# HuiGuanLab/Lite-MKD

Hardware: AMD Instinct MI355X
Metric: episodes/sec (5-way 5-shot, 8x224^2 frames) (higher is better)
Workload: dtype f32

## Files before the change

include/lmkd.h:

```cpp
#ifndef LMKD_H
#define LMKD_H
#ifdef __cplusplus
extern "C" {
#endif

int lmkd_abi_version(void);
const char* lmkd_last_error(void);
int lmkd_device_check(int device);
int lmkd_set_activation_dtype(int mode);
int lmkd_get_activation_dtype(void);

int lmkd_gemm_f32(char layA, char layB, int M, int N, int K, float alpha, const float* A, long lda, long sA,
                  const float* B, long ldb, long sB, float beta, float* C, long ldc, long sC, const float* bias,
                  int relu, int batch, void* stream);
int lmkd_gemm_set_mode(int mode);
int lmkd_gemm_set_tile(int t);
long lmkd_gemm_ticket_words(void);
int lmkd_gemm_f32_splitk(char layA, char layB, int M, int N, int K, float alpha, const float* A, long lda, long sA,
                         const float* B, long ldb, long sB, float beta, float* C, long ldc, long sC, const float* bias,
                         int relu, int batch, void* workspace, long ws_bytes, unsigned* tickets, void* stream);

long lmkd_conv2d_packed_weight_elems(int Cout, int Cin, int Cs, int KH, int KW, int mode);
int lmkd_conv2d_pack_weights(const float* w_oihw, float* wp, int Cout, int Cin, int Cs, int KH, int KW, int mode ,
                             void* stream);
int lmkd_conv2d_fwd_row_tiles(int N, int H, int W, int Cout, int KH, int KW, int stride, int pad);
int lmkd_conv2d_fwd_row_tiles_cs(int N, int H, int W, int Cs, int Cout, int KH, int KW, int stride, int pad);
int lmkd_set_elementwise_wg_per_cu(int n);
int lmkd_conv_set_compute_dtype(int mode);
typedef struct lmkd_amax_desc {
  const void* x_words;
  const void* dy_words;
  void* out_words;
  const void* ref_words;
  int flags;
} lmkd_amax_desc;
#define LMKD_AMAX_FENCED 1
int lmkd_h2_fence_eval(const void* const* words, void* const* refs, int n, int* flags, void* stream);
long lmkd_conv_h2_fallbacks(void);
int lmkd_amax(const float* x, long n, void* word, void* stream);
long lmkd_amax_words(void);
long lmkd_conv2d_plane_elems(int ncols, int Kp);
long lmkd_conv_h2_launches(void);
int lmkd_conv2d_repack_multi(const float* const* ws, void* const* wfs, const int* dims, int n, void* stream);
int lmkd_conv2d_split_weights(const float* wp, void* wf, int ncols, int Kp, void* stream);
int lmkd_conv_get_compute_dtype(void);
int lmkd_conv_set_wgrad_planes(int on);
int lmkd_conv_set_patch(int on);
int lmkd_conv_set_stem_patch(int on);
int lmkd_conv_set_s2_patch(int on);
int lmkd_conv_set_wgrad_win16(int on);
int lmkd_conv_set_wgrad_stem(int on);
int lmkd_conv_set_wgrad_window(int on);
int lmkd_conv_set_patch16(int on);
int lmkd_conv_set_persistent(int on);
int lmkd_conv_set_xcd_mode(int mode);
int lmkd_conv_set_tile(int id);
int lmkd_conv2d_fwd(const float* x, const float* wp_fwd, float* y, float* stat_partial, int N, int H, int W, int Cs, int Cout,
                    int KH, int KW, int stride, int pad, void* stream);
int lmkd_conv2d_fwd_pre(const float* x_raw, const float* pre_stats, const float* wp_fwd, float* y, float* stat_partial, int N, int H,
                        int W, int Cs, int Cout, int KH, int KW, int stride, int pad, void* stream);
int lmkd_conv2d_fwd_bn(const float* x, const float* wp_fwd, float* y, const float* bn_stats, const float* res , int relu,
                       int N, int H, int W, int Cs, int Cout, int KH, int KW, int stride, int pad, void* stream,
                       const lmkd_amax_desc* amax );
int lmkd_conv2d_bwd_data(const float* dy, const float* wp_dgrad, float* dx, int N, int H, int W, int Cin, int Cout, int KH, int KW,
                         int stride, int pad, int accumulate, void* stream);
int lmkd_conv2d_bwd_data_bn_tiles(int N, int H, int W, int Cin, int Cout, int KH, int KW, int stride, int pad);
int lmkd_conv2d_bwd_data_bn(const float* dy, const float* wp_dgrad, float* dx, const float* bn_x, const float* bn_stats, float* part,
                            int N, int H, int W, int Cin, int Cout, int KH, int KW, int stride, int pad, void* stream);
long lmkd_conv2d_bwd_weight_workspace(int N, int H, int W, int Cs, int Cout, int KH, int KW, int stride, int pad);
int lmkd_conv2d_bwd_weight(const float* x, const float* dy, float* dw_oihw, float* workspace, long ws_bytes, int N, int H, int W,
                           int Cs, int Cin, int Cout, int KH, int KW, int stride, int pad, void* stream);
int lmkd_conv2d_bwd_weight_pre(const float* x_raw, const float* pre_stats, const float* dy, float* dw_oihw, float* workspace,
                               long ws_bytes, int N, int H, int W, int Cs, int Cin, int Cout, int KH, int KW, int stride, int pad,
                               void* stream);

int lmkd_conv2d_plan(int kind, int N, int H, int W, int Cs, int Cin, int Cout, int KH, int KW, int stride, int pad, int* info_host);

int lmkd_conv2d_bwd_weight_acc(const float* x, const float* pre_stats, const float* dy, float* dw_oihw, float* workspace, long ws_bytes,
                               int N, int H, int W, int Cs, int Cin, int Cout, int KH, int KW, int stride, int pad, void* stream);

int lmkd_frames_u8_to_nhwc4(const unsigned char* src, float* dst, const int* crop_y, const int* crop_x, const int* flip, int F, int Hs,
                            int Ws, int H, int W, int frames_per_video, void* stream);
int lmkd_resize_plan(int in_size, int out_size, int* bounds_host, int* coeffs_host);
int lmkd_resize_pass_u8(const unsigned char* src, unsigned char* dst, const int* bounds_dev, const int* coeffs_dev, int ksize, long outer,
                        int n_in, int n_out, long inner, void* stream);
int lmkd_frames_resize_crop_nhwc4(const unsigned char* src, float* dst, const int* bounds_h, const int* coeffs_h, int ksize_h,
                                  const int* bounds_v, const int* coeffs_v, int ksize_v, const int* crop_y, const int* crop_x,
                                  const int* flip, int F, int Hs, int Ws, int Hr, int Wr, int H, int W, int frames_per_video, void* stream);
long lmkd_jpeg_desc_bytes(void);
long lmkd_jpeg_pool_bytes(int n);
const char* lmkd_jpeg_reason(int reason);
int lmkd_jpeg_plan(const unsigned char* data, const long long* offsets, int n, void* descs, void* pool, long pool_cap, long long* info,
                   long long* totals);
int lmkd_jpeg_decode(const unsigned char* data, const void* descs, const void* pool, int n, short* coef, unsigned char* planes,
                     unsigned char* out, int* status, long long max_blocks, long long max_pixels, void* stream);
int lmkd_jpeg_decode_host(const unsigned char* data, const void* descs, const void* pool, int n, short* coef, unsigned char* planes,
                          unsigned char* out, int* status);
int lmkd_nchw3_to_nhwc4(const float* x_nchw, float* y_nhwc4, int N, int H, int W, void* stream, void* amax_words);
long lmkd_ticket_words(void);
int lmkd_bn_finalize(const float* partial, int T, int C, long count, const float* gamma, const float* beta, float* running_mean,
                     float* running_var, float momentum, float eps, float* stats, double* scratch, unsigned* tickets, void* stream,
                     const lmkd_amax_desc* amax );
int lmkd_bn_running_update(float* running_mean, float* running_var, const float* stats, int C, float momentum, void* stream);
int lmkd_bn_running_update_multi(float* const* running_mean, float* const* running_var, const float* const* stats_first,
                                 const float* const* stats_second, const int* C, int n, float momentum, void* stream);
int lmkd_bn_running_update_multi_nbt(float* const* running_mean, float* const* running_var, const float* const* stats_first,
                                     const float* const* stats_second, long long* const* num_batches_tracked, const int* C, int n,
                                     float momentum, void* stream);
int lmkd_bn_eval_stats(int C, const float* gamma, const float* beta, const float* running_mean, const float* running_var, float eps,
                       float* stats, void* stream);
int lmkd_bn_apply(const float* x, const float* stats, const float* res, const float* rstats, float* y, long rows, int C, int relu,
                  int res_mode, unsigned* mask_bits, void* stream);
long lmkd_bn_bwd_workspace(int C);
int lmkd_bn_backward(const float* dy, const float* x, const float* yact, const float* stats, const float* gamma, float* dx,
                     float* g_out, float* dgamma, float* dbeta, float* coef, void* workspace, unsigned* tickets, long rows, int C,
                     int mask_mode, int accumulate_param_grads, void* stream);
int lmkd_bn_backward_part(const float* part, int T, const float* dy, const float* x, const float* stats, const float* gamma, float* dx,
                          float* dgamma, float* dbeta, float* coef, void* workspace, unsigned* tickets, long rows, int C,
                          int accumulate_param_grads, void* stream);
int lmkd_relu_backward(const float* dy, const float* y, float* g, long n, void* stream);
int lmkd_bn_relu_maxpool_fwd(const float* x, const float* stats, float* y, unsigned char* idx, float* cmax, int N, int H, int W, int C,
                             void* stream);
int lmkd_maxpool_bwd(const float* dy, const unsigned char* idx, float* g, int N, int H, int W, int C, void* stream);
int lmkd_bn_backward_stats(const float* dy, const float* cmax, const float* stats, const float* gamma, float* dgamma, float* dbeta,
                           float* coef, void* workspace, unsigned* tickets, long pooled_rows, long count, int C, int accumulate_param_grads,
                           void* stream);
int lmkd_stem_unpool_bn_bwd(const float* dy, const unsigned char* idx, const float* c, const float* stats, const float* coef, float* dc,
                            int N, int H, int W, int C, void* stream, const lmkd_amax_desc* amax );
int lmkd_adaptive_maxpool_mean_fwd(const float* x, float* y, int F, int H, int W, int C, void* stream);
int lmkd_adaptive_maxpool_mean_bwd(const float* x, const float* dy, float* dx, int F, int H, int W, int C, void* stream);
long lmkd_colsum_workspace(int C);
// ... 151 lines not shown
```

lite-mkd_amd/csrc/conv.hip:

```cpp
#include "gemm_core.h"
#include <atomic>
#include <mutex>

struct ConvGemmArgs {
  const float* src;
  const float* wpk;
  float* out;
  float* stat_partial;
  int N, Hs, Ws, Cs;
  int Hr, Wr, rows_per_class, tiles_per_class;
  int sh;
  int Ho, Wo, Co, omul;
  int Kp, cps, nclass;
  int n_rt, n_ct, xcd_mode;
  int taps_pm1;
  int grid_step;
  int grid_total;
  int same;
  int halo;
  int accum;
  const float* ep_stats;
  const float* ep_res;
  int ep_relu;
  const float* pre_stats;
// ... 701 lines not shown
  return pr.multiProcessorCount;
}
static int g_conv_persist = 1;
extern "C" int lmkd_conv_set_persistent(int on) { g_conv_persist = on ? 1 : 0; return LMKD_OK; }
template <auto K>
static int persistent_grid(int threads, size_t lds, int total) {
  if (!g_conv_persist) return total;
  static PersistOcc c;
  int occ = 0;
  {
    std::lock_guard<std::mutex> lk(c.mu);
    const int n = c.n.load();
    for (int i = 0; i < n; ++i) if (c.lds[i] == (int)lds) occ = c.occ[i];
    if (!occ) {
      if (hipOccupancyMaxActiveBlocksPerMultiprocessor(&occ, K, threads, lds) != hipSuccess || occ < 1) occ = 1;
      if (n < 8) { c.lds[n] = (int)lds; c.occ[n] = occ; c.n.store(n + 1); }
    }
  }
  const int slots = occ * lmkd_cu_count();
  if (total <= slots) return total;
  const int rounds = cdiv(total, slots);
  const int g = (cdiv(total, rounds) + 7) & ~7;
  return g < total ? g : total;
}

static int g_conv_patch = 1;
extern "C" int lmkd_conv_set_patch(int on) { g_conv_patch = on ? 1 : 0; return LMKD_OK; }
static int patch_halo(const ConvGemmArgs& a) {
  if (!g_conv_patch || !conv_planes() || a.Cs % 32 != 0 || a.sh != 1) return -1;
  const bool plain = a.nclass == 1 && a.Hs == a.Ho && a.Ws == a.Wo;
  const bool classes = a.nclass == 4 && a.Hr == a.Hs && a.Wr == a.Ws;
  if (!plain && !classes) return -1;
  int halo = 0;
  for (int c = 0; c < a.nclass; ++c)
    for (int t = 0; t < a.ntap[c]; ++t) {
      const int sft = a.taps[c][t].dh * a.Ws + a.taps[c][t].dw;
      halo = std::max(halo, sft < 0 ? -sft : sft);
    }
  return halo <= PATCH_HALO_MAX ? halo : -1;
}
static inline bool conv_same_size(int H, int W, int KH, int KW, int stride, int pad) {
  return g_conv_patch && stride == 1 && conv_out(H, KH, stride, pad) == H && conv_out(W, KW, stride, pad) == W && (KH / 2) * W + KW / 2 <= PATCH_HALO_MAX;
}

static int g_conv_s2_patch = 1;
extern "C" int lmkd_conv_set_s2_patch(int on) { g_conv_s2_patch = on ? 1 : 0; return LMKD_OK; }
static int g_patch16 = 1;
extern "C" int lmkd_conv_set_patch16(int on) { g_patch16 = on < 0 ? 0 : (on > 2 ? 2 : on); return LMKD_OK; }

#ifdef LMKD_STAMPS
extern "C" int lmkd_debug_stamps(unsigned long long* host, int zero) {
  if (zero) {
    void* p = nullptr;
    if (hipGetSymbolAddress(&p, HIP_SYMBOL(g_lmkd_stamps)) != hipSuccess) return LMKD_EHIP;
    return hipMemset(p, 0, sizeof(g_lmkd_stamps)) == hipSuccess ? LMKD_OK : LMKD_EHIP;
  }
  return hipMemcpyFromSymbol(host, HIP_SYMBOL(g_lmkd_stamps), sizeof(g_lmkd_stamps)) == hipSuccess ? LMKD_OK : LMKD_EHIP;
}
#endif
static inline int taps_within_one(const ConvGemmArgs& a) {
  for (int c = 0; c < a.nclass; ++c)
    for (int t = 0; t < a.ntap[c]; ++t)
      if (a.taps[c][t].dh < -1 || a.taps[c][t].dh > 1 || a.taps[c][t].dw < -1 || a.taps[c][t].dw > 1) return 0;
  return 1;
}

static bool fwd_s2_patch_ok(int N, int H, int W, int Cs, int Cout, int KH, int KW, int stride, int pad) {
  if (!(g_conv_s2_patch && g_patch16 && g_conv_patch && conv_nprod(g_lmkd_act_bf16) >= 6) || Cs % 32 != 0 || stride != 2 || KH != 3 ||
      KW != 3 || pad != 1 || H % 2 != 0 || W % 2 != 0 || W / 2 + 1 > PATCH_HALO_MAX)
    return false;
  const int id = pick_conv_cfg((long)N * (H / 2) * (W / 2), 1, Cout, true);
  return id == 11 || id == 12;
}

static int g_conv_stem_patch = 1;
extern "C" int lmkd_conv_set_stem_patch(int on) { g_conv_stem_patch = on ? 1 : 0; return LMKD_OK; }
static int stem_patch_pitch(int W, int Cs, int Cout, int KH, int KW, int stride, int pad) {
  if (!g_conv_stem_patch || !conv_planes() || Cs != 4 || KH != 7 || KW != 7 || stride != 2 || pad != 3 || Cout > 64) return 0;
  const int Wo = conv_out(W, KW, stride, pad);
  int wp = std::max(2 * Wo + 6, W + 3);
  wp += wp & 1;
  return (2 * Wo <= 256 && wp <= STEM_MAX_WP) ? wp : 0;
}

enum class ConvFam : unsigned char {
  Tile,
  Gather,
  Patch,
  Patch16,
  Patch1p,
  Stem,
};
enum ConvIO : unsigned char { IO_PLAIN, IO_PRE, IO_EP, IO_ACT16, IO_BNB };
struct ConvPlan {
  ConvFam fam;
  unsigned char io;
  bool src2;
  bool smallc;
  bool bnb_form;
  bool amax_pass;
  int stats;
  int tile;
  int nprod;
  int nclass, xcd;
  int halo;
  int seg_m0, seg_t0, tiles_per_class, n_rt, n_ct;
  int grid;
  int lds;
};

static void fwd_geometry(ConvGemmArgs& a, int N, int H, int W, int Cs, int Cout, int KH, int KW, int stride, int pad, int seg_n0) {
  memset(&a, 0, sizeof(a));
  const int KWp = kw_padded(Cs, KW);
  a.N = N; a.Hs = H; a.Ws = W; a.Cs = Cs;
  a.Ho = conv_out(H, KH, stride, pad); a.Wo = conv_out(W, KW, stride, pad); a.Co = Cout;
  a.Hr = a.Ho; a.Wr = a.Wo; a.rows_per_class = N * a.Ho * a.Wo; a.tiles_per_class = cdiv(a.rows_per_class, 128);
  a.seg_m0 = seg_n0 * a.Ho * a.Wo;
  a.sh = stride; a.omul = 1; a.nclass = 1;
  a.Kp = KH * KWp * Cs;
  a.div_hw = make_fastdiv(a.Hr * a.Wr); a.div_w = make_fastdiv(a.Wr);
  if (Cs == 4) {
    a.cps = 1;
    if (KH > LMKD_MAX_TAPS) return;
    a.ntap[0] = KH;
    for (int kh = 0; kh < KH; ++kh) a.taps[0][kh] = Tap{kh - pad, -pad, kh * KWp * Cs};
  } else {
    a.cps = Cs / 32;
    if (KH * KW > LMKD_MAX_TAPS) return;
    a.ntap[0] = KH * KW;
    for (int kh = 0; kh < KH; ++kh)
      for (int kw = 0; kw < KW; ++kw) a.taps[0][kh * KW + kw] = Tap{kh - pad, kw - pad, (kh * KWp + kw) * Cs};
  }
}

static void dgrad_geometry(ConvGemmArgs& a, int N, int H, int W, int Cin, int Cout, int KH, int KW, int stride, int pad, int seg_n0) {
  memset(&a, 0, sizeof(a));
  const int Ho = conv_out(H, KH, stride, pad), Wo = conv_out(W, KW, stride, pad);
  a.N = N; a.Hs = Ho; a.Ws = Wo; a.Cs = Cout;
  a.Ho = H; a.Wo = W; a.Co = Cin;
  a.Kp = KH * KW * Cout; a.cps = Cout / 32;
  a.sh = 1;
  const bool fits = KH * KW <= LMKD_MAX_TAPS;
  if (stride == 1) {
    a.nclass = 1; a.omul = 1; a.Hr = H; a.Wr = W;
    int nt = 0;
    for (int kh = 0; kh < KH && fits; ++kh)
      for (int kw = 0; kw < KW; ++kw) a.taps[0][nt++] = Tap{pad - kh, pad - kw, (kh * KW + kw) * Cout};
    a.ntap[0] = nt;
  } else {
    a.nclass = 4; a.omul = 2; a.Hr = (H + 1) / 2; a.Wr = (W + 1) / 2;
    for (int c = 0; c < 4 && fits; ++c) {
      const int ph = c >> 1, pw = c & 1;
      int nt = 0;
      for (int kh = 0; kh < KH; ++kh) {
        if (((ph + pad - kh) & 1) != 0) continue;
        for (int kw = 0; kw < KW; ++kw) {
          if (((pw + pad - kw) & 1) != 0) continue;
          const int nh = ph + pad - kh, nw = pw + pad - kw;
          a.taps[c][nt++] = Tap{nh >= 0 ? nh / 2 : -((-nh) / 2), nw >= 0 ? nw / 2 : -((-nw) / 2), (kh * KW + kw) * Cout};
        }
      }
      a.ntap[c] = nt;
    }
  }
  a.rows_per_class = N * a.Hr * a.Wr;
  a.seg_m0 = seg_n0 * a.Hr * a.Wr;
  a.tiles_per_class = cdiv(a.rows_per_class, 128);
  a.div_hw = make_fastdiv(a.Hr * a.Wr); a.div_w = make_fastdiv(a.Wr);
}

static ConvPlan plan_conv(const ConvGemmArgs& a, int halo, bool same, bool smallc, int stats, bool src2) {
  ConvPlan p;
  memset(&p, 0, sizeof(p));
  const bool act16 = g_lmkd_act_bf16;
  const int ncols = a.Co;
  p.io = a.ep_stats ? IO_EP : act16 ? IO_ACT16 : a.pre_stats ? IO_PRE : a.bnb_x ? IO_BNB : IO_PLAIN;
  p.src2 = src2; p.smallc = smallc; p.stats = stats; p.nclass = a.nclass; p.halo = halo;
  int id = pick_conv_cfg(a.rows_per_class, a.nclass, ncols, same);
  if (conv_planes() && !(stats == 2 && smallc)) {
    if (halo < 0) {
      id = id == 10 || id == 13 || id == 14 ? 7 : (id == 11 ? 9 : (id == 12 ? 8 : id));
      p.fam = ConvFam::Gather;
      p.nprod = conv_nprod(act16);
    } else if (id == 13 || id == 14) {
      p.fam = ConvFam::Patch1p;
      p.nprod = 1;
    } else {
      const bool h2 = conv_nprod(act16, a.h2_xw && !a.ep_stats) == 3;
      const bool h2_on_32 = g_patch16 == 1 && id == 11 && ncols <= 64 && h2 && !src2;
      const bool p16 = (id == 11 || id == 12) && g_patch16 && conv_nprod(act16) >= 6;
      p.bnb_form = p16 && a.nclass == 1 && ncols % 4 == 0;
      if (p16 && !h2_on_32) {
        p.fam = ConvFam::Patch16;
        p.nprod = conv_nprod(false, a.h2_xw);
      } else {
        p.fam = ConvFam::Patch;
        p.nprod = h2 ? 3 : conv_nprod(act16);
      }
    }
  } else {
    p.fam = ConvFam::Tile;
    if (id != 1 && id != 2 && id != 3 && id != 5 && id != 6) id = 4;
  }
  p.tile = id;
  const int bm = cfg_bm(id);
  p.seg_m0 = (a.seg_m0 <= 0 || a.seg_m0 >= a.rows_per_class) ? a.rows_per_class : a.seg_m0;
  p.seg_t0 = cdiv(p.seg_m0, bm);
  p.tiles_per_class = p.seg_t0 + cdiv(a.rows_per_class - p.seg_m0, bm);
  p.n_rt = a.nclass * p.tiles_per_class;
  p.n_ct = cdiv(ncols, cfg_bn(id));
  p.xcd = g_xcd_mode != 0 && p.n_ct >= 8 && (p.n_ct & 7) == 0;
  p.grid = xcd_grid(p.n_rt, p.n_ct, p.xcd);
  if (p.fam == ConvFam::Patch || p.fam == ConvFam::Patch16 || p.fam == ConvFam::Patch1p)
    p.lds = (int)patch_lds_bytes(bm, halo, p.nprod == 1 ? 1 : (p.nprod == 3 && p.fam == ConvFam::Patch ? 2 : 3));
  p.amax_pass = !act16 && p.fam != ConvFam::Patch16 && !(p.fam == ConvFam::Patch && p.nprod == 3);
  return p;
}

static ConvPlan plan_fwd(const ConvGemmArgs& a, int KH, int KW, int pad) {
  const int N = a.N, H = a.Hs, W = a.Ws, Cs = a.Cs, Cout = a.Co, stride = a.sh;
  if (const int wp = a.ep_stats ? 0 : stem_patch_pitch(W, Cs, Cout, KH, KW, stride, pad)) {
    ConvPlan p;
    memset(&p, 0, sizeof(p));
    p.fam = ConvFam::Stem;
    p.io = g_lmkd_act_bf16 ? IO_ACT16 : IO_PLAIN;
    p.tile = 14; p.nclass = 1; p.halo = wp;
    p.nprod = conv_nprod(g_lmkd_act_bf16, a.h2_xw);
    const int seg_n0 = a.seg_m0 > 0 && a.seg_m0 < a.rows_per_class ? a.seg_m0 / (a.Ho * a.Wo) : N;
    p.seg_t0 = seg_n0 * cdiv(a.Ho, 2);
    p.n_rt = p.tiles_per_class = p.grid = N * cdiv(a.Ho, 2);
    p.n_ct = 1;
    p.lds = (p.nprod == 1 ? 1 : 3) * 9 * wp * 8;
    return p;
  }
  const int stats = a.ep_stats ? 2 : (a.stat_partial ? 1 : 0);
  if (!a.pre_stats && fwd_s2_patch_ok(N, H, W, Cs, Cout, KH, KW, stride, pad)) return plan_conv(a, a.Wo + 1, true, false, stats, true);
  const int halo = Cs == 4 || !a.ntap[0] ? -1 : patch_halo(a);
  return plan_conv(a, halo, conv_same_size(H, W, KH, KW, stride, pad), Cs == 4, stats, false);
}

static ConvPlan plan_dgrad(const ConvGemmArgs& a) {
  const int halo = a.ntap[0] ? patch_halo(a) : -1;
  return plan_conv(a, halo, halo >= 0, false, 0, false);
}

static void fwd_src2_args(ConvGemmArgs& a, int W, int KWp) {
  const int Cs = a.Cs;
  a.src2 = 1; a.s2_ncls = 4; a.s2_wfull = W;
  a.Hs = a.Ho; a.Ws = a.Wo; a.sh = 1;
  static const int order[4][2] = {{1, 1}, {1, 0}, {0, 1}, {0, 0}};
  int nt = 0;
  for (int c = 0; c < 4; ++c) {
    const int sph = order[c][0], spw = order[c][1];
    a.s2_t0[c] = nt;
    a.s2_off[c] = (sph * W + spw) * Cs;
    for (int kh = 0; kh < 3; ++kh) {
      if (((kh - 1) & 1) != sph) continue;
      for (int kw = 0; kw < 3; ++kw) {
        if (((kw - 1) & 1) != spw) continue;
        a.taps[0][nt++] = Tap{(kh - 1 - sph) / 2, (kw - 1 - spw) / 2, (kh * KWp + kw) * Cs};
      }
    }
  }
  a.s2_t0[4] = nt;
  a.ntap[0] = nt;
}

template <int... Ps, class F>
static inline void with_nprod(int n, F&& f) {
  if (n == 3) ++g_h2_launches;
  (void)((n == Ps ? (f(std::integral_constant<int, Ps>{}), true) : false) || ...);
}

template <class Cfg, int NPROD, bool PRE, int IO>
static void launch_patch_instance(ConvGemmArgs& a, const ConvPlan& p, hipStream_t s) {
  constexpr auto K = conv_patch_x3_kernel<Cfg, NPROD, PRE, IO>;
  lds_attr_once<K>((int)patch_lds_bytes(Cfg::BM, PATCH_HALO_MAX, NPROD == 1 ? 1 : 3));
  a.grid_total = p.grid;
  a.grid_step = NPROD == 3 ? persistent_grid<K>(Cfg::THREADS, p.lds, p.grid) : p.grid;
  hipLaunchKernelGGL((conv_patch_x3_kernel<Cfg, NPROD, PRE, IO>), dim3(a.grid_step), dim3(Cfg::THREADS), p.lds, s, a);
}
template <class Cfg, bool ONE_PLANE = false>
static void launch_patch(ConvGemmArgs& a, const ConvPlan& p, hipStream_t s) {
  if constexpr (ONE_PLANE) {
    if (p.io == IO_EP) launch_patch_instance<Cfg, 1, false, 4>(a, p, s);
    else if (p.io == IO_ACT16) launch_patch_instance<Cfg, 1, false, 3>(a, p, s);
    else if (p.io == IO_PRE) launch_patch_instance<Cfg, 1, true, 0>(a, p, s);
    else launch_patch_instance<Cfg, 1, false, 0>(a, p, s);
  } else {
    if (p.io == IO_EP) with_nprod<1, 6, 9>(p.nprod, [&](auto np) { launch_patch_instance<Cfg, np, false, 4>(a, p, s); });
    else if (p.io == IO_ACT16) launch_patch_instance<Cfg, 1, false, 3>(a, p, s);
    else if (p.io == IO_PRE) with_nprod<1, 3, 6, 9>(p.nprod, [&](auto np) { launch_patch_instance<Cfg, np, true, 0>(a, p, s); });
    else with_nprod<1, 3, 6, 9>(p.nprod, [&](auto np) { launch_patch_instance<Cfg, np, false, 0>(a, p, s); });
  }
}
template <class Cfg, int NPROD, bool PRE, bool EP, bool SRC2 = false, bool BNB = false>
static void launch_patch16_instance(const ConvGemmArgs& a, const ConvPlan& p, hipStream_t s) {
  lds_attr_once<conv_patch16_x3_kernel<Cfg, NPROD, PRE, EP, SRC2, BNB>>((int)patch_lds_bytes(Cfg::BM, PATCH_HALO_MAX, 3));
  hipLaunchKernelGGL((conv_patch16_x3_kernel<Cfg, NPROD, PRE, EP, SRC2, BNB>), dim3(p.grid), dim3(Cfg::THREADS), p.lds, s, a);
}
template <class Cfg>
static void launch_patch16(const ConvGemmArgs& a, const ConvPlan& p, hipStream_t s) {
  with_nprod<3, 6, 9>(p.nprod, [&](auto np) {
    if (p.src2 && p.io == IO_EP) launch_patch16_instance<Cfg, np, false, true, true>(a, p, s);
    else if (p.src2) launch_patch16_instance<Cfg, np, false, false, true>(a, p, s);
    else if (p.io == IO_EP) launch_patch16_instance<Cfg, np, false, true>(a, p, s);
    else if (p.io == IO_PRE) launch_patch16_instance<Cfg, np, true, false>(a, p, s);
    else if (p.io == IO_BNB) launch_patch16_instance<Cfg, np, false, false, false, true>(a, p, s);
    else launch_patch16_instance<Cfg, np, false, false>(a, p, s);
  });
}
template <class Cfg, bool SMALLC>
static void launch_gather(const ConvGemmArgs& a, const ConvPlan& p, hipStream_t s) {
  const dim3 grid(p.grid), block(Cfg::THREADS);
  if (p.io == IO_ACT16) {
    if constexpr (SMALLC) hipLaunchKernelGGL((conv_gemm_x3_kernel<Cfg, true, true, 1, false, 2>), grid, block, 0, s, a);
    else hipLaunchKernelGGL((conv_gemm_x3_kernel<Cfg, false, true, 1, false, 3>), grid, block, 0, s, a);
    return;
  }
  if constexpr (!SMALLC) {
    if (p.io == IO_EP) {
      with_nprod<1, 6, 9>(p.nprod, [&](auto np) { hipLaunchKernelGGL((conv_gemm_x3_kernel<Cfg, false, true, np, false, 4>), grid, block, 0, s, a); });
      return;
    }
    if (p.io == IO_PRE) {
      with_nprod<1, 6, 9>(p.nprod, [&](auto np) { hipLaunchKernelGGL((conv_gemm_x3_kernel<Cfg, false, true, np, true>), grid, block, 0, s, a); });
      return;
    }
  }
  with_nprod<1, 6, 9>(p.nprod, [&](auto np) { hipLaunchKernelGGL((conv_gemm_x3_kernel<Cfg, SMALLC, true, np>), grid, block, 0, s, a); });
}
template <class Cfg>
static void launch_tile(const ConvGemmArgs& a, const ConvPlan& p, hipStream_t s) {
  const dim3 grid(p.grid), block(Cfg::THREADS);
  if (p.smallc) {
    if (p.stats == 2) hipLaunchKernelGGL((conv_gemm_kernel<Cfg, true, 2, false>), grid, block, 0, s, a);
    else if (p.stats == 1) hipLaunchKernelGGL((conv_gemm_kernel<Cfg, true, 1, false>), grid, block, 0, s, a);
    else hipLaunchKernelGGL((conv_gemm_kernel<Cfg, true, 0, false>), grid, block, 0, s, a);
  } else if (p.stats == 2) hipLaunchKernelGGL((conv_gemm_kernel<Cfg, false, 2, false>), grid, block, 0, s, a);
  else if (p.stats == 1 && p.io == IO_PRE)
    hipLaunchKernelGGL((conv_gemm_kernel<Cfg, false, 1, false, true>), grid, block, 0, s, a);
  else if (p.stats == 1) hipLaunchKernelGGL((conv_gemm_kernel<Cfg, false, 1, false>), grid, block, 0, s, a);
  else hipLaunchKernelGGL((conv_gemm_kernel<Cfg, false, 0, false>), grid, block, 0, s, a);
}

static int launch_conv(ConvGemmArgs& a, const ConvPlan& p, hipStream_t s) {
  if (p.fam == ConvFam::Stem) {
    a.halo = p.halo;
    a.n_rt = p.n_rt; a.n_ct = 1;
    const dim3 grid(p.grid), block(512);
    if (p.io == IO_ACT16) hipLaunchKernelGGL((conv_stem_patch_kernel<1, true, 2>), grid, block, p.lds, s, a);
    else with_nprod<1, 3, 6, 9>(p.nprod, [&](auto np) { hipLaunchKernelGGL((conv_stem_patch_kernel<np, false, 2>), grid, block, p.lds, s, a); });
    LMKD_CHECK_LAUNCH("conv_stem_patch_kernel");
    return LMKD_OK;
  }
  a.seg_m0 = p.seg_m0; a.seg_t0 = p.seg_t0; a.tiles_per_class = p.tiles_per_class;
  a.n_rt = p.n_rt; a.n_ct = p.n_ct; a.xcd_mode = p.xcd;
  switch (p.fam) {
    case ConvFam::Tile:
      switch (p.tile) {
        case 1: launch_tile<TileCfg<128, 128, 2, 2>>(a, p, s); break;
        case 2: launch_tile<TileCfg<128, 64, 2, 2>>(a, p, s); break;
        case 3: launch_tile<TileCfg<64, 64, 2, 2>>(a, p, s); break;
        case 5: launch_tile<TileCfg<128, 128, 2, 4>>(a, p, s); break;
        case 6: launch_tile<TileCfg<128, 64, 4, 2>>(a, p, s); break;
        default: launch_tile<TileCfg<64, 128, 2, 2>>(a, p, s); break;
      }
      LMKD_CHECK_LAUNCH("conv_gemm_kernel");
      return LMKD_OK;
    case ConvFam::Gather:
      switch (p.tile * 2 + p.smallc) {
        case 14: launch_gather<X3Cfg<256, 64, 4, 2>, false>(a, p, s); break;
        case 15: launch_gather<X3Cfg<256, 64, 4, 2>, true>(a, p, s); break;
        case 16: launch_gather<X3Cfg<128, 128, 2, 4>, false>(a, p, s); break;
        case 17: launch_gather<X3Cfg<128, 128, 2, 4>, true>(a, p, s); break;
        case 19: launch_gather<X3Cfg<128, 64, 4, 2>, true>(a, p, s); break;
        default: launch_gather<X3Cfg<128, 64, 4, 2>, false>(a, p, s); break;
      }
      LMKD_CHECK_LAUNCH("conv_gemm_x3_kernel");
      return LMKD_OK;
    default: break;
  }
  a.taps_pm1 = taps_within_one(a);
  a.halo = p.halo;
  switch (p.tile) {
    case 7: launch_patch<X3Cfg<256, 64, 4, 2>>(a, p, s); break;
    case 8: launch_patch<X3Cfg<128, 128, 2, 4>>(a, p, s); break;
    case 10: launch_patch<X3Cfg<256, 128, 2, 4>>(a, p, s); break;
    case 11:
      if (p.fam == ConvFam::Patch16) launch_patch16<X3Cfg<128, 64, 2, 2, 3>>(a, p, s);
      else launch_patch<X3Cfg<128, 64, 2, 2, 3>>(a, p, s);
      break;
    case 12:
      if (p.fam == ConvFam::Patch16) launch_patch16<X3Cfg<128, 128, 2, 2, 2>>(a, p, s);
      else launch_patch<X3Cfg<128, 128, 2, 2, 2>>(a, p, s);
      break;
    case 13: launch_patch<X3Cfg<256, 128, 2, 2, 2>, true>(a, p, s); break;
    case 14: launch_patch<X3Cfg<256, 64, 2, 2, 2>, true>(a, p, s); break;
    default: launch_patch<X3Cfg<128, 64, 4, 2>>(a, p, s); break;
  }
  LMKD_CHECK_LAUNCH("conv_patch_x3_kernel");
  return LMKD_OK;
}

extern "C" int lmkd_conv2d_fwd_row_tiles_seg(int N, int H, int W, int Cs, int Cout, int KH, int KW, int stride, int pad, int seg_n0, int* tiles0);
extern "C" int lmkd_conv2d_fwd_row_tiles_cs(int N, int H, int W, int Cs, int Cout, int KH, int KW, int stride, int pad) {
  return lmkd_conv2d_fwd_row_tiles_seg(N, H, W, Cs, Cout, KH, KW, stride, pad, 0, nullptr);
}
extern "C" int lmkd_conv2d_fwd_row_tiles_seg(int N, int H, int W, int Cs, int Cout, int KH, int KW, int stride, int pad, int seg_n0, int* tiles0) {
  if (seg_n0 <= 0 || seg_n0 >= N) seg_n0 = 0;
  ConvGemmArgs a;
  fwd_geometry(a, N, H, W, Cs, Cout, KH, KW, stride, pad, seg_n0);
  const ConvPlan p = plan_fwd(a, KH, KW, pad);
  if (tiles0) *tiles0 = p.seg_t0;
  return p.tiles_per_class;
}
extern "C" int lmkd_conv2d_fwd_row_tiles(int N, int H, int W, int Cout, int KH, int KW, int stride, int pad) {
  return lmkd_conv2d_fwd_row_tiles_cs(N, H, W, 32, Cout, KH, KW, stride, pad);
}

static int conv2d_fwd_impl(const float* x, const float* wp, float* y, float* stat_partial, const float* ep_stats,
                           const float* ep_res, int ep_relu, int N, int H, int W, int Cs, int Cout, int KH, int KW, int stride,
                           int pad, void* stream, const float* pre_stats = nullptr, int seg_n0 = 0, const lmkd_amax_desc* am = nullptr) {
  LMKD_REQUIRE(x && wp && y, "lmkd_conv2d_fwd: null pointer");
  if (seg_n0 <= 0 || seg_n0 >= N) seg_n0 = 0;
  LMKD_REQUIRE(!seg_n0 || (conv_planes() && !ep_stats), "lmkd_conv2d_fwd_seg: two frame segments exist in the bf16-plane modes (training / plain forward)");
  LMKD_REQUIRE(aligned16(x) && aligned16(wp), "lmkd_conv2d_fwd: x / packed weights must be 16-byte aligned");
  LMKD_REQUIRE(Cs % 32 == 0 || Cs == 4, "lmkd_conv2d_fwd: channel count %d must be 4 (padded stem) or a multiple of 32", Cs);
  LMKD_REQUIRE(N > 0 && H > 0 && W > 0 && Cout > 0, "lmkd_conv2d_fwd: empty tensor");
  const bool smallc = Cs == 4;
  const int KWp = kw_padded(Cs, KW);
  LMKD_REQUIRE(!smallc || KWp == 8, "lmkd_conv2d_fwd: padded-stem path needs KW <= 8");
// ... 495 lines not shown
```

lite-mkd_amd/csrc/conv_stem.h:

```cpp
#pragma once

#define STEM_MAX_WP 240

template <int NPROD, bool OUT16, int OR>
__global__ __launch_bounds__(256 * OR) void conv_stem_patch_kernel(ConvGemmArgs a) {
  constexpr int NPL = NPROD == 1 ? 1 : (NPROD == 3 ? 2 : 3);
  constexpr int NTHR = 256 * OR;
  using Cfg = X3Cfg<128 * OR, 64, 4 * OR, 1>;
  using LB = X3FragB<Cfg::TN, NPL>;
  constexpr int KH = 7, PR = 2 * (OR - 1) + KH;
  extern __shared__ __attribute__((aligned(16))) unsigned char psm[];
  __shared__ int s_out[Cfg::BM];
  __shared__ float s_red[Cfg::WM * Cfg::BN * 2];
  const int tid = threadIdx.x, lane = tid & 63, wave = tid >> 6;
  const int rt = blockIdx.x;
  const int pairs = (a.Ho + OR - 1) / OR;
  const int n = rt / pairs, oh0 = (rt - n * pairs) * OR;
  const int WP = a.halo;
  const int plane_bytes = PR * WP * 8;
  const int ih0 = 2 * oh0 - 3;
  float h2_sx = 1.f, h2_ix = 1.f, h2_iw = 1.f;
  if constexpr (NPROD == 3) {
    h2_sx = h2_scale(amax_read(a.h2_xw, (a.seg_m0 > 0 && (long)n * a.Ho * a.Wo >= a.seg_m0) ? 1 : 0));
    h2_ix = 1.f / h2_sx;
    h2_iw = 1.f / h2_scale(*reinterpret_cast<const unsigned*>(reinterpret_cast<const unsigned short*>(a.wpk) + wpl_amax((long)a.Co * a.Kp)));
  }
  {
    static_assert(STEM_MAX_WP <= 256, "one thread per patch column");
    constexpr int RSTEP = NTHR / 256, NIT = (PR + RSTEP - 1) / RSTEP;
    const __amdgpu_buffer_rsrc_t rs = x3_rsrc(a.src, (long)a.N * a.Hs * a.Ws * 16);
    const int pc = tid & 255, iw = pc - 3;
    u32x4 rp[NIT];
#pragma unroll
    for (int it = 0; it < NIT; ++it) {
      const int pr = (tid >> 8) + RSTEP * it, ih = ih0 + pr;
      const bool ok = pr < PR && (unsigned)ih < (unsigned)a.Hs && (unsigned)iw < (unsigned)a.Ws;
      rp[it] = __builtin_amdgcn_raw_buffer_load_b128(rs, ok ? (unsigned)(((n * a.Hs + ih) * a.Ws + iw) * 16) : X3_OOB, 0, 0);
    }
#pragma unroll
    for (int it = 0; it < NIT; ++it) {
      const int pr = (tid >> 8) + RSTEP * it;
      if (pr >= PR || pc >= WP) continue;
      const float4 v = make_float4(__uint_as_float(rp[it].x), __uint_as_float(rp[it].y), __uint_as_float(rp[it].z), __uint_as_float(rp[it].w));
      unsigned char* d = psm + (pr * WP + pc) * 8;
      if (NPL == 1) {
        *reinterpret_cast<uint2*>(d) = x3_round4(v);
      } else if constexpr (NPROD == 3) {
        uint2 q0, q1;
        h2_split4(v, h2_sx, q0, q1);
        *reinterpret_cast<uint2*>(d) = q0;
        *reinterpret_cast<uint2*>(d + plane_bytes) = q1;
      } else {
        uint2 q0, q1, q2;
        x3_split4(v, q0, q1, q2);
        *reinterpret_cast<uint2*>(d) = q0;
        *reinterpret_cast<uint2*>(d + plane_bytes) = q1;
        *reinterpret_cast<uint2*>(d + 2 * plane_bytes) = q2;
      }
    }
  }
  const int npix = OR * a.Wo;
  for (int r = tid; r < Cfg::BM; r += NTHR) {
    const int orow = r / a.Wo, ow = r - orow * a.Wo;
    s_out[r] = (r < npix && oh0 + orow < a.Ho) ? ((n * a.Ho + oh0 + orow) * a.Wo + ow) * a.Co : -1;
  }
  const int m = wave * 32 + (lane & 31);
  const bool active = __builtin_amdgcn_readfirstlane(wave * 32) < npix;
  int a_off = 0;
  {
    const int mm = m < npix ? m : 0;
    const int orow = mm / a.Wo, ow = mm - orow * a.Wo;
    a_off = ((2 * orow) * WP + 2 * ow + 2 * (lane >> 5)) * 8;
  }
  LB lb;
  lb.init(a.wpk, a.Co, a.Kp, 0, lane);
  f32x16 acc[1][Cfg::TN];
#pragma unroll
  for (int j = 0; j < Cfg::TN; ++j)
#pragma unroll
    for (int e = 0; e < 16; ++e) acc[0][j][e] = 0.f;
  u32x4 rb0[LB::NR], rb1[LB::NR];
  if (active) lb.load(0, rb0);
  __syncthreads();
  if (active) {
    auto step = [&](int kh, u32x4 (&rb)[LB::NR], u32x4 (&rbn)[LB::NR]) {
      if (kh + 1 < KH) lb.load((kh + 1) * 32, rbn);
      bf16x8 av[2][NPL];
#pragma unroll
      for (int g = 0; g < 2; ++g)
#pragma unroll
        for (int p = 0; p < NPL; ++p) av[g][p] = *reinterpret_cast<const bf16x8*>(psm + a_off + (kh * WP + 4 * g) * 8 + p * plane_bytes);
#pragma unroll
      for (int g = 0; g < 2; ++g)
#pragma unroll
        for (int j = 0; j < Cfg::TN; ++j) {
          f32x16 c = acc[0][j];
          if constexpr (NPROD == 1) {
            c = __builtin_amdgcn_mfma_f32_32x32x16_bf16(av[g][0], x3_as_bf16(rb[j * 2 + g]), c, 0, 0, 0);
          } else if constexpr (NPROD == 3) {
            const bf16x8 b0 = x3_as_bf16(rb[j * 4 + g * 2 + 0]), b1 = x3_as_bf16(rb[j * 4 + g * 2 + 1]);
            c = __builtin_amdgcn_mfma_f32_32x32x16_f16(__builtin_bit_cast(f16x8, av[g][1]), __builtin_bit_cast(f16x8, b0), c, 0, 0, 0);
            c = __builtin_amdgcn_mfma_f32_32x32x16_f16(__builtin_bit_cast(f16x8, av[g][0]), __builtin_bit_cast(f16x8, b1), c, 0, 0, 0);
            c = __builtin_amdgcn_mfma_f32_32x32x16_f16(__builtin_bit_cast(f16x8, av[g][0]), __builtin_bit_cast(f16x8, b0), c, 0, 0, 0);
          } else {
            const bf16x8 b0 = x3_as_bf16(rb[j * 6 + g * 3 + 0]), b1 = x3_as_bf16(rb[j * 6 + g * 3 + 1]), b2 = x3_as_bf16(rb[j * 6 + g * 3 + 2]);
            if (NPROD == 9) {
              c = __builtin_amdgcn_mfma_f32_32x32x16_bf16(av[g][2], b2, c, 0, 0, 0);
              c = __builtin_amdgcn_mfma_f32_32x32x16_bf16(av[g][1], b2, c, 0, 0, 0);
              c = __builtin_amdgcn_mfma_f32_32x32x16_bf16(av[g][2], b1, c, 0, 0, 0);
            }
            c = __builtin_amdgcn_mfma_f32_32x32x16_bf16(av[g][1], b1, c, 0, 0, 0);
            c = __builtin_amdgcn_mfma_f32_32x32x16_bf16(av[g][0], b2, c, 0, 0, 0);
            c = __builtin_amdgcn_mfma_f32_32x32x16_bf16(av[g][2], b0, c, 0, 0, 0);
            c = __builtin_amdgcn_mfma_f32_32x32x16_bf16(av[g][0], b1, c, 0, 0, 0);
            c = __builtin_amdgcn_mfma_f32_32x32x16_bf16(av[g][1], b0, c, 0, 0, 0);
            c = __builtin_amdgcn_mfma_f32_32x32x16_bf16(av[g][0], b0, c, 0, 0, 0);
          }
          acc[0][j] = c;
        }
    };
    step(0, rb0, rb1); step(1, rb1, rb0); step(2, rb0, rb1); step(3, rb1, rb0); step(4, rb0, rb1); step(5, rb1, rb0); step(6, rb0, rb1);
  }
#pragma unroll
  for (int e = 0; e < 16; ++e)
    if (s_out[wave * 32 + acc_row(e, lane)] < 0)
#pragma unroll
      for (int j = 0; j < Cfg::TN; ++j) acc[0][j][e] = 0.f;
  if constexpr (NPROD == 3) {
#pragma unroll
    for (int j = 0; j < Cfg::TN; ++j)
#pragma unroll
      for (int e = 0; e < 16; ++e) acc[0][j][e] = acc[0][j][e] * h2_ix * h2_iw;
  }
  x3_epilogue<Cfg, true, OUT16>(a, acc, s_out, s_red, rt, 0, wave, 0, lane, tid);
}
```

Measured before the change: 51.37.

## Add persistent rolling-window stem conv kernel reusing input rows across output pairs

Adds a persistent 7x7 stride-2 stem convolution kernel that processes strips of eight output row-pairs per block. It keeps a ring buffer of input rows in LDS, so only four new rows are loaded per pair instead of reloading all nine. Weights are held in registers, or in LDS for the higher split-product modes, and the next rows are prefetched while the MFMAs run. The aim is to cut redundant input loads, per-tile weight reloads and launch overhead, at the cost of more LDS and register pressure and a serial dependency inside each strip.

After: 51.83 (median of 6 runs). Within noise of the previous version (+0.9%).

```diff
diff --git a/include/lmkd.h b/include/lmkd.h
--- a/include/lmkd.h
+++ b/include/lmkd.h
@@ -47,6 +47,7 @@
 int lmkd_conv_set_wgrad_planes(int on);
 int lmkd_conv_set_patch(int on);
 int lmkd_conv_set_stem_patch(int on);
+int lmkd_conv_set_stem_roll(int on);
 int lmkd_conv_set_s2_patch(int on);
 int lmkd_conv_set_wgrad_win16(int on);
 int lmkd_conv_set_wgrad_stem(int on);
diff --git a/lite-mkd_amd/csrc/conv.hip b/lite-mkd_amd/csrc/conv.hip
--- a/lite-mkd_amd/csrc/conv.hip
+++ b/lite-mkd_amd/csrc/conv.hip
@@ -807,6 +807,9 @@
   wp += wp & 1;
   return (2 * Wo <= 256 && wp <= STEM_MAX_WP) ? wp : 0;
 }
+static int g_conv_stem_roll = 1;
+extern "C" int lmkd_conv_set_stem_roll(int on) { g_conv_stem_roll = on ? 1 : 0; return LMKD_OK; }
+static inline int stem_planes(int nprod) { return nprod == 1 ? 1 : (nprod == 3 ? 2 : 3); }
 
 enum class ConvFam : unsigned char {
   Tile,
@@ -955,7 +958,7 @@
     p.seg_t0 = seg_n0 * cdiv(a.Ho, 2);
     p.n_rt = p.tiles_per_class = p.grid = N * cdiv(a.Ho, 2);
     p.n_ct = 1;
-    p.lds = (p.nprod == 1 ? 1 : 3) * 9 * wp * 8;
+    p.lds = stem_planes(p.nprod) * 9 * wp * 8;
     return p;
   }
   const int stats = a.ep_stats ? 2 : (a.stat_partial ? 1 : 0);
@@ -1069,10 +1072,30 @@
   else hipLaunchKernelGGL((conv_gemm_kernel<Cfg, false, 0, false>), grid, block, 0, s, a);
 }
 
+template <int NPROD, bool OUT16, int R, bool WLDS>
+static void launch_stem_roll(const ConvGemmArgs& a, const ConvPlan& p, hipStream_t s) {
+  constexpr auto K = conv_stem_roll_kernel<NPROD, OUT16, R, WLDS>;
+  constexpr int NPL = NPROD == 1 ? 1 : (NPROD == 3 ? 2 : 3);
+  constexpr int wbytes = WLDS ? stem_wlds_bytes<NPL>() : 0;
+  lds_attr_once<K>(NPL * R * STEM_MAX_WP * 8 + wbytes);
+  const size_t lds = (size_t)NPL * R * p.halo * 8 + wbytes;
+  const int strips = a.N * cdiv(cdiv(a.Ho, 2), STEM_STRIP);
+  hipLaunchKernelGGL((conv_stem_roll_kernel<NPROD, OUT16, R, WLDS>), dim3(persistent_grid<K>(512, lds, strips)), dim3(512), lds, s, a);
+}
+
 static int launch_conv(ConvGemmArgs& a, const ConvPlan& p, hipStream_t s) {
   if (p.fam == ConvFam::Stem) {
     a.halo = p.halo;
     a.n_rt = p.n_rt; a.n_ct = 1;
+    if (g_conv_stem_roll && !a.accum) {
+      if (p.io == IO_ACT16) launch_stem_roll<1, true, 13, false>(a, p, s);
+      else if (p.nprod == 1) launch_stem_roll<1, false, 13, false>(a, p, s);
+      else if (p.nprod == 3) { ++g_h2_launches; launch_stem_roll<3, false, 13, false>(a, p, s); }
+      else if (p.nprod == 6) launch_stem_roll<6, false, 9, true>(a, p, s);
+      else launch_stem_roll<9, false, 9, true>(a, p, s);
+      LMKD_CHECK_LAUNCH("conv_stem_roll_kernel");
+      return LMKD_OK;
+    }
     const dim3 grid(p.grid), block(512);
     if (p.io == IO_ACT16) hipLaunchKernelGGL((conv_stem_patch_kernel<1, true, 2>), grid, block, p.lds, s, a);
     else with_nprod<1, 3, 6, 9>(p.nprod, [&](auto np) { hipLaunchKernelGGL((conv_stem_patch_kernel<np, false, 2>), grid, block, p.lds, s, a); });
diff --git a/lite-mkd_amd/csrc/conv_stem.h b/lite-mkd_amd/csrc/conv_stem.h
--- a/lite-mkd_amd/csrc/conv_stem.h
+++ b/lite-mkd_amd/csrc/conv_stem.h
@@ -1,6 +1,24 @@
 #pragma once
 
 #define STEM_MAX_WP 240
+
+template <int NPROD>
+__device__ __forceinline__ void stem_store_px(unsigned char* d, int plane_bytes, const float4& v, float sx) {
+  if constexpr (NPROD == 1) {
+    *reinterpret_cast<uint2*>(d) = x3_round4(v);
+  } else if constexpr (NPROD == 3) {
+    uint2 q0, q1;
+    h2_split4(v, sx, q0, q1);
+    *reinterpret_cast<uint2*>(d) = q0;
+    *reinterpret_cast<uint2*>(d + plane_bytes) = q1;
+  } else {
+    uint2 q0, q1, q2;
+    x3_split4(v, q0, q1, q2);
+    *reinterpret_cast<uint2*>(d) = q0;
+    *reinterpret_cast<uint2*>(d + plane_bytes) = q1;
+    *reinterpret_cast<uint2*>(d + 2 * plane_bytes) = q2;
+  }
+}
 
 template <int NPROD, bool OUT16, int OR>
 __global__ __launch_bounds__(256 * OR) void conv_stem_patch_kernel(ConvGemmArgs a) {
@@ -42,21 +60,7 @@
       const int pr = (tid >> 8) + RSTEP * it;
       if (pr >= PR || pc >= WP) continue;
       const float4 v = make_float4(__uint_as_float(rp[it].x), __uint_as_float(rp[it].y), __uint_as_float(rp[it].z), __uint_as_float(rp[it].w));
-      unsigned char* d = psm + (pr * WP + pc) * 8;
-      if (NPL == 1) {
-        *reinterpret_cast<uint2*>(d) = x3_round4(v);
-      } else if constexpr (NPROD == 3) {
-        uint2 q0, q1;
-        h2_split4(v, h2_sx, q0, q1);
-        *reinterpret_cast<uint2*>(d) = q0;
-        *reinterpret_cast<uint2*>(d + plane_bytes) = q1;
-      } else {
-        uint2 q0, q1, q2;
-        x3_split4(v, q0, q1, q2);
-        *reinterpret_cast<uint2*>(d) = q0;
-        *reinterpret_cast<uint2*>(d + plane_bytes) = q1;
-        *reinterpret_cast<uint2*>(d + 2 * plane_bytes) = q2;
-      }
+      stem_store_px<NPROD>(psm + (pr * WP + pc) * 8, plane_bytes, v, h2_sx);
     }
   }
   const int npix = OR * a.Wo;
@@ -134,3 +138,201 @@
   }
   x3_epilogue<Cfg, true, OUT16>(a, acc, s_out, s_red, rt, 0, wave, 0, lane, tid);
 }
+
+#define STEM_STRIP 8
+
+template <int NPROD>
+__device__ __forceinline__ f32x16 stem_products(f32x16 c, const bf16x8* av , const bf16x8* b ) {
+  if constexpr (NPROD == 1) {
+    c = __builtin_amdgcn_mfma_f32_32x32x16_bf16(av[0], b[0], c, 0, 0, 0);
+  } else if constexpr (NPROD == 3) {
+    c = __builtin_amdgcn_mfma_f32_32x32x16_f16(__builtin_bit_cast(f16x8, av[1]), __builtin_bit_cast(f16x8, b[0]), c, 0, 0, 0);
+    c = __builtin_amdgcn_mfma_f32_32x32x16_f16(__builtin_bit_cast(f16x8, av[0]), __builtin_bit_cast(f16x8, b[1]), c, 0, 0, 0);
+    c = __builtin_amdgcn_mfma_f32_32x32x16_f16(__builtin_bit_cast(f16x8, av[0]), __builtin_bit_cast(f16x8, b[0]), c, 0, 0, 0);
+  } else {
+    if (NPROD == 9) {
+      c = __builtin_amdgcn_mfma_f32_32x32x16_bf16(av[2], b[2], c, 0, 0, 0);
+      c = __builtin_amdgcn_mfma_f32_32x32x16_bf16(av[1], b[2], c, 0, 0, 0);
+      c = __builtin_amdgcn_mfma_f32_32x32x16_bf16(av[2], b[1], c, 0, 0, 0);
+    }
+    c = __builtin_amdgcn_mfma_f32_32x32x16_bf16(av[1], b[1], c, 0, 0, 0);
+    c = __builtin_amdgcn_mfma_f32_32x32x16_bf16(av[0], b[2], c, 0, 0, 0);
+    c = __builtin_amdgcn_mfma_f32_32x32x16_bf16(av[2], b[0], c, 0, 0, 0);
+    c = __builtin_amdgcn_mfma_f32_32x32x16_bf16(av[0], b[1], c, 0, 0, 0);
+    c = __builtin_amdgcn_mfma_f32_32x32x16_bf16(av[1], b[0], c, 0, 0, 0);
+    c = __builtin_amdgcn_mfma_f32_32x32x16_bf16(av[0], b[0], c, 0, 0, 0);
+  }
+  return c;
+}
+
+template <int NPL> constexpr int stem_wlds_bytes() { return 2 * 14 * NPL * 1024; }
+
+template <int NPROD, bool OUT16, int R, bool WLDS>
+__global__ __launch_bounds__(512) void conv_stem_roll_kernel(ConvGemmArgs a) {
+  constexpr int NPL = NPROD == 1 ? 1 : (NPROD == 3 ? 2 : 3);
+  constexpr int KH = 7, NEWR = 4, FIRSTR = 9;
+  static_assert(R >= FIRSTR, "the ring holds a tile's nine rows");
+  using LB = X3FragB<1, NPL>;
+  extern __shared__ __attribute__((aligned(16))) unsigned char psm[];
+  __shared__ float s_red[2][8 * 64 * 2];
+  const int tid = threadIdx.x, lane = tid & 63, wave = tid >> 6;
+  const int rg = wave >> 1, cb = wave & 1;
+  const int WP = a.halo;
+  const int row_bytes = WP * 8, plane_bytes = R * row_bytes;
+  const int pairs = (a.Ho + 1) / 2, strips = (pairs + STEM_STRIP - 1) / STEM_STRIP, nstrips = a.N * strips;
+  const int npix = 2 * a.Wo;
+  const __amdgpu_buffer_rsrc_t rs = x3_rsrc(a.src, (long)a.N * a.Hs * a.Ws * 16);
+  const int pc = tid & 255, iw = pc - 3, half = tid >> 8;
+
+  int a_col[2];
+  bool a_row1[2], act[2];
+#pragma unroll
+  for (int i = 0; i < 2; ++i) {
+    const int m = (2 * rg + i) * 32 + (lane & 31);
+    const int mm = m < npix ? m : 0;
+    const int orow = mm / a.Wo, ow = mm - orow * a.Wo;
+    a_col[i] = (2 * ow + 2 * (lane >> 5)) * 8;
+    a_row1[i] = orow != 0;
+    act[i] = __builtin_amdgcn_readfirstlane((2 * rg + i) * 32) < npix;
+  }
+
+  LB lb;
+  lb.init(a.wpk, a.Co, a.Kp, cb * 32, lane);
+  u32x4 wreg[WLDS ? 1 : KH][LB::NR];
+  unsigned char* const wsm = psm + NPL * plane_bytes;
+  if constexpr (WLDS) {
+    constexpr int PER_NT = 14 * NPL * 64;
+    for (int i = tid; i < 2 * PER_NT; i += 512) {
+      const bool ok = (i >= PER_NT ? 32 : 0) < a.Co;
+      const u32x4 v = __builtin_amdgcn_raw_buffer_load_b128(lb.rs, ok ? (unsigned)(i * 16) : X3_OOB, 0, 0);
+      *reinterpret_cast<u32x4*>(wsm + i * 16) = v;
+    }
+  } else {
+#pragma unroll
+    for (int kh = 0; kh < KH; ++kh) lb.load(kh * 32, wreg[kh]);
+  }
+  float h2_iw = 1.f;
+  if constexpr (NPROD == 3)
+    h2_iw = 1.f / h2_scale(*reinterpret_cast<const unsigned*>(reinterpret_cast<const unsigned short*>(a.wpk) + wpl_amax((long)a.Co * a.Kp)));
+
+  int par = 0;
+  for (int sid = blockIdx.x; sid < nstrips; sid += gridDim.x) {
+    const int n = sid / strips, p0 = (sid - n * strips) * STEM_STRIP;
+    const int pend = p0 + STEM_STRIP < pairs ? p0 + STEM_STRIP : pairs;
+    float h2_sx = 1.f, h2_ix = 1.f;
+    if constexpr (NPROD == 3) {
+      h2_sx = h2_scale(amax_read(a.h2_xw, (a.seg_m0 > 0 && (long)n * a.Ho * a.Wo >= a.seg_m0) ? 1 : 0));
+      h2_ix = 1.f / h2_sx;
+    }
+    auto load_row = [&](int ih) {
+      const bool ok = (unsigned)ih < (unsigned)a.Hs && (unsigned)iw < (unsigned)a.Ws;
+      return __builtin_amdgcn_raw_buffer_load_b128(rs, ok ? (unsigned)(((n * a.Hs + ih) * a.Ws + iw) * 16) : X3_OOB, 0, 0);
+    };
+    auto store_row = [&](int slot, const u32x4& r) {
+      const float4 v = make_float4(__uint_as_float(r.x), __uint_as_float(r.y), __uint_as_float(r.z), __uint_as_float(r.w));
+      stem_store_px<NPROD>(psm + slot * row_bytes + pc * 8, plane_bytes, v, h2_sx);
+    };
+    {
+      constexpr int NIT = (FIRSTR + 1) / 2;
+      u32x4 rp[NIT];
+#pragma unroll
+      for (int it = 0; it < NIT; ++it) rp[it] = load_row(half + 2 * it < FIRSTR ? 4 * p0 - 3 + half + 2 * it : -1);
+#pragma unroll
+      for (int it = 0; it < NIT; ++it)
+        if (half + 2 * it < FIRSTR && pc < WP) store_row(half + 2 * it, rp[it]);
+    }
+    __syncthreads();
+    int s0 = 0;
+    for (int p = p0; p < pend; ++p) {
+      const int oh0 = 2 * p, rt = n * pairs + p;
+      const bool more = p + 1 < pend;
+      u32x4 rn[NEWR / 2];
+      if (more) {
+#pragma unroll
+        for (int it = 0; it < NEWR / 2; ++it) rn[it] = load_row(4 * p - 3 + FIRSTR + half + 2 * it);
+      }
+      f32x16 acc[2];
+#pragma unroll
+      for (int i = 0; i < 2; ++i)
+#pragma unroll
+        for (int e = 0; e < 16; ++e) acc[i][e] = 0.f;
+      auto mm = [&](int i, int kh) {
+        if (!act[i]) return;
+        const int ro0 = ((s0 + kh) % R) * row_bytes, ro1 = ((s0 + kh + 2) % R) * row_bytes;
+        const unsigned char* ap = psm + a_col[i] + (a_row1[i] ? ro1 : ro0);
+        bf16x8 av[2][NPL], bv[2][NPL];
+#pragma unroll
+        for (int g = 0; g < 2; ++g)
+#pragma unroll
+          for (int q = 0; q < NPL; ++q) {
+            av[g][q] = *reinterpret_cast<const bf16x8*>(ap + g * 32 + q * plane_bytes);
+            if constexpr (WLDS) bv[g][q] = *reinterpret_cast<const bf16x8*>(wsm + (((cb * 14 + kh * 2 + g) * NPL + q) * 64 + lane) * 16);
+            else bv[g][q] = x3_as_bf16(wreg[kh][g * NPL + q]);
+          }
+#pragma unroll
+        for (int g = 0; g < 2; ++g) acc[i] = stem_products<NPROD>(acc[i], av[g], bv[g]);
+      };
+      constexpr int ESZ = OUT16 ? 2 : 4;
+      const int nvalid = (oh0 + 1 < a.Ho ? 2 : 1) * a.Wo;
+      const int col = cb * 32 + (lane & 31);
+      const long tile_off = ((long)(n * a.Ho + oh0) * a.Wo) * a.Co;
+      const __amdgpu_buffer_rsrc_t ro = x3_rsrc(reinterpret_cast<unsigned char*>(a.out) + tile_off * ESZ, (long)nvalid * a.Co * ESZ);
+      int coe = a.Co * ESZ;
+      asm volatile("" : "+s"(coe));
+      float* const red = s_red[par];
+      auto epi = [&](int i) {
+        const int rb = 2 * rg + i, r_lane = rb * 32 + 4 * (lane >> 5);
+        const unsigned v0 = col < a.Co ? (unsigned)(r_lane * coe + col * ESZ) : 0x80000000u;
+        float s1 = 0.f, s2 = 0.f;
+#pragma unroll
+        for (int e = 0; e < 16; ++e) {
+          const int dr = (e & 3) + 8 * (e >> 2);
+          float v = r_lane + dr < nvalid ? acc[i][e] : 0.f;
+          if constexpr (NPROD == 3) v = v * h2_ix * h2_iw;
+          if constexpr (OUT16) {
+            const lmkd_bf16_t b = f32_to_bf16(v);
+            __builtin_amdgcn_raw_buffer_store_b16(__builtin_bit_cast(short, b), ro, v0 + (unsigned)(dr * coe), 0, 0);
+            v = bf16_to_f32(b);
+          } else {
+            __builtin_amdgcn_raw_buffer_store_b32(__float_as_uint(v), ro, v0 + (unsigned)(dr * coe), 0, 0);
+          }
+          s1 += v;
+          s2 = fmaf(v, v, s2);
+        }
+        const float t1 = s1 + __shfl_xor(s1, 32, 64), t2 = s2 + __shfl_xor(s2, 32, 64);
+        if (lane < 32) {
+          red[(rb * 64 + col) * 2 + 0] = t1;
+          red[(rb * 64 + col) * 2 + 1] = t2;
+        }
+      };
+#pragma unroll
+      for (int kh = 0; kh < KH; ++kh) {
+        mm(0, kh);
+        mm(1, kh);
+        if constexpr (!WLDS) __builtin_amdgcn_sched_barrier(0);
+      }
+      if constexpr (R < FIRSTR + NEWR) __syncthreads();
+      if (more) {
+#pragma unroll
+        for (int it = 0; it < NEWR / 2; ++it)
+          if (pc < WP) store_row((s0 + FIRSTR + half + 2 * it) % R, rn[it]);
+      }
+      epi(0);
+      epi(1);
+      __syncthreads();
+      if (tid < 64 && tid < a.Co && a.stat_partial) {
+        float t1 = 0.f, t2 = 0.f;
+#pragma unroll
+        for (int w = 0; w < 8; ++w) {
+          t1 += red[(w * 64 + tid) * 2 + 0];
+          t2 += red[(w * 64 + tid) * 2 + 1];
+        }
+        float* q = a.stat_partial + ((long)rt * a.Co + tid) * 2;
+        q[0] = t1;
+        q[1] = t2;
+      }
+      s0 = (s0 + NEWR) % R;
+      par ^= 1;
+    }
+  }
+}
```
